# DrSleep/nas-segm-pytorch

Hardware: AMD Instinct MI355X
Metric: images/sec (fwd+bwd+optimizer step) WACV arch0 2048x1024 bs=4/GPU (higher is better)
Workload: dtype f32

## Files before the change

### include/nasseg.h

```cpp
#ifndef NASSEG_H
#define NASSEG_H

#include <stdint.h>

#ifdef __cplusplus
extern "C" {
#endif

const char* nasseg_last_error(void);
int nasseg_abi_version(void);
int nasseg_device_count(void);

int nasseg_dw_pack_weight(const float* w, float* wt, int C, int K, int flip, void* stream);
int nasseg_dwconv(const float* x, const float* wt, float* y, const float* in_scale,
                  const float* in_shift, int in_act, const float* scale, const float* shift, int act,
                  int B, int H, int W, int C, int Ho, int Wo, int K, int stride, int pad, int dil,
                  int transposed, float* stats, void* stream);
int nasseg_dwconv_strip_ok(int K, int stride, int dil);
int64_t nasseg_dwconv_stats_blocks(int B, int C, int Ho, int Wo, int K, int stride, int dil);
int nasseg_dwconv_bwd_data_bn(const float* dy, const float* wt, float* g, const float* z,
                              const float* scale, const float* shift, const float* mean,
                              const float* invstd, int act, int B, int H, int W, int C, int Ho,
                              int Wo, int K, int stride, int pad, int dil, int transposed,
                              float* stats, void* stream);
// ... 7 lines not shown
                         int B, int H, int W, int C, int Ho, int Wo, int K, int stride, int pad, int dil, float* stats,
                         void* stream);
int64_t nasseg_dwconv_wgrad_workspace(int B, int C, int Ho, int Wo, int K);
int nasseg_dwconv_wgrad(const float* x, const float* dy, float* dw, float* ws,
                        const float* in_scale, const float* in_shift, int in_act, int B, int H, int W,
                        int C, int Ho, int Wo, int K, int stride, int pad, int dil, void* stream);

int nasseg_dw_wgrad_lds(int v);

int64_t nasseg_sepconv_blocks(int B, int C, int Ho, int Wo, int N, int K, int stride, int dil);
int nasseg_sepconv_fwd(const float* x, const float* wdw, const float* wpw, float* zdw, float* y,
                       const float* in_scale, const float* in_shift, int in_act,
                       const float* out_scale, const float* out_shift, int out_act, int B, int H,
                       int W, int C, int Ho, int Wo, int N, int K, int stride, int pad, int dil,
                       float* stats, void* stream);

int64_t nasseg_irdw_rows(int B, int H, int W, int K, int C, int stride, int backward);
int64_t nasseg_irdw_config(int B, int H, int W, int K, int C, int stride, int backward);
int64_t nasseg_irdw_stats_workspace(int K);
int nasseg_irdw_stats(const float* x, const float* w1, const float* in_scale, const float* in_shift, int in_act, int B,
                      int H, int W, int K, int C, float eps, float momentum, const float* gamma, const float* beta,
                      float* mean, float* invstd, float* scale, float* shift, float* running_mean, float* running_var,
                      int64_t* num_batches_tracked, float* ws, void* stream);
int nasseg_irdw_fwd(const float* x, const float* w1, const float* wdw, float* z2, const float* in_scale,
                    const float* in_shift, int in_act, const float* bn1_scale, const float* bn1_shift, int act1,
                    int B, int H, int W, int K, int C, int Ho, int Wo, int stride, float* stats, void* stream);
int nasseg_irdw_bwd(const float* x, const float* w1, const float* g, const float* z2, const float* wdw,
                    int wdw_flipped, float* ge, float* dw, float* ws, const float* in_scale, const float* in_shift,
                    int in_act, const float* bn1_scale, const float* bn1_shift, const float* bn1_mean,
                    const float* bn1_invstd, int act1, const float* bn2_scale, const float* bn2_shift,
                    const float* bn2_mean, const float* bn2_invstd, const float* bn2_sums, int bn2_train, int bn2_act,
                    int B, int H, int W, int K, int C, int Ho, int Wo, int stride, float* stats, void* stream);

int nasseg_conv_pack_weight(const float* w, float* wp, int N, int K, int kh, int kw, int mode,
                            void* stream);
int nasseg_pack_weights(int count, const float* const* w, float* const* wp, const int* dims,
                        void* stream);
int nasseg_conv_fwd_pack_mode(int K, int kh, int kw);
int nasseg_conv_fwd(const float* x, int ldx, const float* wp, float* y, int ldy,
                    const float* in_scale, const float* in_shift, int in_act,
                    const float* out_scale, const float* out_shift, int out_act, const float* res,
                    int ldres, int B, int Hs, int Ws, int K, int Ho, int Wo, int N, int kh, int kw,
                    int stride, int pad, int dil, int transposed, float* stats, void* stream);
int64_t nasseg_conv_fwd_stats_blocks(int B, int Ho, int Wo, int N, int K, int pointwise);
int64_t nasseg_conv_fwd_stats_rows(int B, int Ho, int Wo, int N, int K, int kh, int kw, int stride, int pad, int dil);
int64_t nasseg_conv_pw_min_pixels(int64_t v);
int nasseg_conv_pwn_mode(int v);
int nasseg_conv_deep_k(int v);
int nasseg_pool_strip(int v);
int64_t nasseg_conv_pointwise_kernel(int B, int Ho, int Wo, int N, int K, int pointwise);
int64_t nasseg_conv_fwd_lds3x3(int B, int Ho, int Wo, int N, int K, int kh, int kw, int stride, int pad, int dil,
                               int with_stats);
int nasseg_conv_bwd_data_bn(const float* dy, int lddy, const float* wp, float* g, int ldg,
                            const float* z, int ldz, const float* scale, const float* shift,
                            const float* mean, const float* invstd, int act, int B, int Hs, int Ws,
                            int K, int Ho, int Wo, int N, int kh, int kw, int stride, int pad,
                            int dil, float* stats, void* stream);
int nasseg_conv_wgrad_lds3x3(int B, int Hs, int Ws, int K, int Ho, int Wo, int N, int kh, int kw, int stride,
                             int pad, int dil);
int64_t nasseg_conv_wgrad_workspace(int B, int Ho, int Wo, int N, int K, int kh, int kw);
int nasseg_wgrad_finalize_many(int count, const float* const* partial, float* const* dw,
                               const int* dims, void* stream);
int nasseg_conv_wgrad_many(int count, const int64_t* desc, void* stream);
int nasseg_dwconv_wgrad_many(int count, const int64_t* desc, void* stream);

int nasseg_conv_wgrad_bn(const float* x, int ldx, const float* g, int ldg, const float* z, int ldz, float* dz,
                         int lddz, float* dw, float* ws, const float* in_scale, const float* in_shift, int in_act,
                         const float* bn_scale, const float* bn_shift, const float* bn_mean, const float* bn_invstd,
                         const float* bn_sums, int bn_train, int bn_act, int B, int H, int W, int K, int N, void* stream);
int nasseg_conv_wgrad_bn_flat(const float* x, int ldx, const float* g, int ldg, const float* z, int ldz, float* dw,
                              float* ws, const float* bn_scale, const float* bn_shift, const float* bn_mean,
                              const float* bn_invstd, const float* bn_sums, int bn_train, int bn_act, int B, int Hs,
                              int Ws, int K, int Ho, int Wo, int N, int kh, int kw, int stride, int pad, int dil,
                              void* stream);
int nasseg_dwconv_wgrad_bn(const float* x, const float* g, const float* z, float* dz, float* dw, float* ws,
                           const float* in_scale, const float* in_shift, int in_act, const float* bn_scale, const float* bn_shift,
                           const float* bn_mean, const float* bn_invstd, const float* bn_sums, int bn_train, int bn_act,
                           int B, int H, int W, int C, int Ho, int Wo, int K, int stride, int pad, int dil,
                           void* stream);
int64_t nasseg_conv_pw_bwd_slabs(int B, int H, int W, int K, int N);
int64_t nasseg_conv_pw_bwd_reads_z(int B, int H, int W, int K, int N);
int64_t nasseg_conv_pw_bwd_kernel_id(int B, int H, int W, int K, int N, int z_null);
int64_t nasseg_conv_pw_bwd_rz_min_pixels(int64_t v);
int nasseg_conv_pw_bwd_bn(const float* x, const float* g, const float* z, const float* wb, float* dx, float* dw,
                          float* ws, const float* in_scale, const float* in_shift, int in_act, int dx_act,
                          const float* bn_scale, const float* bn_shift, const float* bn_mean, const float* bn_invstd,
                          const float* bn_sums, int bn_train, int bn_act, int B, int H, int W, int K, int N,
                          const float* in_mean, const float* in_invstd, float* dx_stats, const float* dx_res,
                          void* stream);
int nasseg_conv_wgrad(const float* x, int ldx, const float* dy, int lddy, float* dw, float* ws,
                      const float* in_scale, const float* in_shift, int in_act, int B, int Hs,
                      int Ws, int K, int Ho, int Wo, int N, int kh, int kw, int stride, int pad,
                      int dil, void* stream);

int64_t nasseg_colred_workspace(int S, int64_t R, int C);
int nasseg_colred(int mode, const float* a, int64_t lda, const float* b, int64_t ldb,
                  const float* c, int64_t ldc, float* out, float* ws, int S, int64_t R, int C,
                  float mul, void* stream);
int nasseg_bn_stats(const float* x, int64_t ldx, int64_t M, int C, float eps, float momentum,
                    const float* gamma, const float* beta, float* mean, float* invstd,
                    float* scale, float* shift, float* running_mean, float* running_var,
                    int64_t* num_batches_tracked, float* ws, void* stream);
int nasseg_bn_finalize(float* partial, int nblk, int64_t M, int C, float eps, float momentum,
                       const float* gamma, const float* beta, float* mean, float* invstd,
                       float* scale, float* shift, float* running_mean, float* running_var,
                       int64_t* num_batches_tracked, void* stream);
int nasseg_bn_eval_params(int C, float eps, const float* gamma, const float* beta,
                          const float* running_mean, const float* running_var, float* mean,
                          float* invstd, float* scale, float* shift, void* stream);
int nasseg_bn_bwd_reduce(const float* dy, int64_t lddy, const float* x, int64_t ldx, int64_t M,
                         int C, const float* scale, const float* shift, const float* mean,
                         const float* invstd, int act, float* sums, float* ws, void* stream);
int nasseg_rows_sum(float* partial, int nblk, int cols, float* out, void* stream);
int nasseg_bn_bwd_apply(const float* dy, const float* x, const float* scale, const float* shift,
                        const float* mean, const float* invstd, const float* sums, int64_t M,
                        int C, int train, int act, float* dx, void* stream);
int64_t nasseg_colred_rows(int S, int64_t R, int C);
int64_t nasseg_bn_bwd_apply_rows_max_bytes(void);
int nasseg_bn_bwd_reduce_rows(const float* dy, int64_t lddy, const float* x, int64_t ldx, int64_t M, int C,
                              const float* scale, const float* shift, const float* mean, const float* invstd, int act,
                              float* rows, void* stream);
int nasseg_bn_bwd_apply_rows(const float* dy, const float* x, const float* scale, const float* shift, const float* mean,
                             const float* invstd, const float* rows, int nrows, float* sums_out, int64_t M, int C,
                             int train, int act, float* dx, void* stream);

int nasseg_affine_act(const float* x, const float* scale, const float* shift, const float* res,
                      float* y, int64_t n, int C, int act, void* stream);
int nasseg_axpby(const float* a, const float* b, const float* alpha, const float* beta, float* y,
                 int64_t n, int C, int act, void* stream);
int nasseg_add_act2(const float* xa, const float* sa, const float* ha, int act_a, const float* ca, const float* xb,
                    const float* sb, const float* hb, int act_b, const float* cb, float* y, int64_t n, int C,
                    void* stream);
int nasseg_act_bwd(const float* dy, const float* ref, float* dx, int64_t n, int act, void* stream);
int nasseg_fill(float* y, int64_t n, float v, void* stream);
int nasseg_chan_copy(const float* x, int64_t ldx, int xoff, float* y, int64_t ldy, int yoff,
                     const float* mref, int64_t ldm, int moff, int64_t P, int C, int act, int mact,
                     void* stream);
int nasseg_chan_fold(const float* dy, float* dx, int64_t P, int C, int rep, void* stream);
int nasseg_gather_rows(const void* src, const int64_t* idx, void* dst, int n, int64_t row_bytes,
                       int64_t n_src, void* stream);

int nasseg_pool_fwd(int mode, const float* x, float* y, uint8_t* idx, int B, int H, int W, int C,
                    int Ho, int Wo, int K, int stride, int pad, void* stream);
int nasseg_pool_bwd(int mode, const float* dy, const uint8_t* idx, float* dx, int B, int H, int W,
                    int C, int Ho, int Wo, int K, int stride, int pad, void* stream);
int64_t nasseg_maxpool_bn_bwd_blocks(int B, int H, int W, int C, int K, int stride, int pad);
int nasseg_maxpool_bn_fwd(const float* z, const float* scale, const float* shift, float* y, uint8_t* idx,
                          int B, int H, int W, int C, int Ho, int Wo, int stride, int pad, void* stream);
int nasseg_maxpool_bn_bwd(const float* dy, const uint8_t* idx, const float* z, const float* mean,
                          const float* invstd, float* g, float* stats, int B, int H, int W, int C, int Ho,
                          int Wo, int stride, int pad, void* stream);

int64_t nasseg_cat_src_blocks(int B, int Ho, int Wo, int C);
int nasseg_psum_bwd(const float* dy, const float* za, const float* tsa, int act_a, const float* ca, float* ga,
                    float* part_a, const float* zb, const float* tsb, int act_b, const float* cb, float* gb,
                    float* part_b, float* cpart, int B, int H, int W, int C, void* stream);
int nasseg_grad_junction(const float* g0, const float* g1, const float* g2, const float* g3, const float* g4,
                         const float* g5, const float* g6, const float* g7, int n, const float* z, const float* tstats,
                         int act, float* out, float* part, int B, int H, int W, int C, void* stream);
int nasseg_cat_src_fwd(const float* x, const float* scale, const float* shift, int act, float* y, int64_t ldy,
                       int yoff, float* stats, int B, int Hi, int Wi, int C, int Ho, int Wo, void* stream);
int nasseg_cat_src_bwd(const float* du, const float* slab, int64_t ld, int off, const float* sscale,
                       const float* smean, const float* sinvstd, const float* sums, int train, const float* z,
                       const float* tstats, int act, float* g, float* part, int B, int Ho, int Wo, int C, int Hi,
                       int Wi, void* stream);
int nasseg_bilinear_bwd_act(const float* dy, int64_t lddy, int dyoff, const float* z, const float* scale,
// ... 302 lines not shown
```

### nas-segm-pytorch_amd/csrc/conv_pwbwd.hip

```cpp
#include <atomic>
#include <cstdlib>
#include <type_traits>

#include "conv_common.h"

#if NASSEG_FP32_ONLY
std::atomic<int64_t> g_pw_rz_min_pixels{1 << 18};
#else
extern std::atomic<int64_t> g_pw_rz_min_pixels;
#endif

namespace {

#ifndef NASSEG_PW_CHUNK
#define NASSEG_PW_CHUNK 3
#endif
#ifndef NASSEG_PW_RECOMPUTE_Z
#define NASSEG_PW_RECOMPUTE_Z 1
#endif
constexpr int kPwTile = 64;
constexpr int kPwMaxTiles = 24;

struct PwArgs {
  const act_t* x;
  const act_t* g;
  const act_t* z;
  act_t* dx;
  float* partial;
  const float* wb;
  const float* in_scale;
  const float* in_shift;
  int in_act;
  const float* bn_scale;
  const float* bn_shift;
  const float* bn_mean;
  const float* bn_invstd;
  const float* bn_sums;
  int bn_train, bn_act;
  float invM;
  int dx_act;
  const float* in_mean;
  const float* in_invstd;
  float* dx_stats;
  const act_t* dx_res;
  int K, N, KP, NP;
  int M, pix_per_slab;
};

__device__ __forceinline__ float4 act_mask_of(float4 v, int act) {
  const float hi = act == NASSEG_ACT_RELU6 ? 6.f : __builtin_inff();
  return make_float4((v.x > 0.f && v.x < hi) ? 1.f : 0.f, (v.y > 0.f && v.y < hi) ? 1.f : 0.f,
                     (v.z > 0.f && v.z < hi) ? 1.f : 0.f, (v.w > 0.f && v.w < hi) ? 1.f : 0.f);
}

__host__ __device__ constexpr int pw_lsn(int NT) { return NT * 16 + 4; }
__host__ __device__ constexpr int pw_lsk(int KT) { return KT * 16 + 4; }
__host__ __device__ constexpr int pw_lds_floats(int NT, int KT, bool WL) {
  return kPwTile * (pw_lsn(NT) + pw_lsk(KT)) + 4 * NT * 16 + 2 * KT * 16 + (WL ? KT * 16 * pw_lsn(NT) : 0);
}
__host__ __device__ constexpr bool pw_weight_in_lds(int NT, int KT) {
  return pw_lds_floats(NT, KT, true) * 4 <= (72 << 10);
}
__host__ __device__ constexpr bool pw_prefetch(int NT, int KT) { return NT * KT <= 18; }

template <int NT, int KT, bool PRO, bool DXS = false, bool RZ_ = false>
__global__ __launch_bounds__(256) void conv_pw_bwd_kernel(PwArgs a) {
  extern __shared__ float smem[];
  constexpr int LSN = pw_lsn(NT), LSK = pw_lsk(KT), NPc = NT * 16, KPc = KT * 16;
  constexpr bool WL = pw_weight_in_lds(NT, KT), PF = pw_prefetch(NT, KT);
  constexpr bool RZ = WL && RZ_;
  float* dzt = smem;
  float* xt = dzt + kPwTile * LSN;
  float* ca = xt + kPwTile * LSK;
  float* cb = ca + NPc;
  float* cd = cb + NPc;
  float* cs = cd + NPc;
  float* psc = cs + NPc;
  float* psh = psc + KPc;
  float* wl = psh + KPc;
  float* xraw = wl + (WL ? KPc * LSN : 0);
  const int tid = threadIdx.x;
  const int lane = tid & 63, wave = tid >> 6;
  const int j = lane & 15, kg = lane >> 4;
  const int N = a.N, K = a.K;

  for (int n = tid; n < NPc; n += 256) {
    float va = 0.f, vb = 0.f, vd = 0.f, vs = 0.f;
    if (n < N) {
      const float sc = a.bn_scale[n];
      va = sc;
      vs = a.bn_act ? a.bn_shift[n] : 0.f;
      if (a.bn_train) {
        const float is = a.bn_invstd[n], mu = a.bn_mean[n];
        const float s0 = a.bn_sums[n] * a.invM, s1 = a.bn_sums[N + n] * a.invM;
        vb = -sc * is * s1;
        vd = sc * (mu * is * s1 - s0);
      }
    }
    ca[n] = va; cb[n] = vb; cd[n] = vd; cs[n] = vs;
  }
  for (int k = tid; k < KPc; k += 256) {
    psc[k] = (PRO && a.in_scale && k < K) ? a.in_scale[k] : 1.f;
    psh[k] = (PRO && a.in_shift && k < K) ? a.in_shift[k] : 0.f;
  }
  if (WL) {
    for (int it = tid; it < KPc * (NPc / 4); it += 256) {
      const int k = it / (NPc / 4), n = (it - k * (NPc / 4)) * 4;
      const float4 v = keep_if(ld4(a.wb + (int64_t)(k < K ? k : 0) * N + (n < N ? n : 0)), k < K && n < N);
      *reinterpret_cast<float4*>(&wl[k * LSN + n]) = v;
    }
  }
  const ActSel pact = act_sel(a.in_act);

  f32x4 acc2[NT][KT];
#pragma unroll
  for (int nt = 0; nt < NT; ++nt)
#pragma unroll
    for (int kt = 0; kt < KT; ++kt) acc2[nt][kt] = (f32x4){0.f, 0.f, 0.f, 0.f};

  const int p_begin = blockIdx.x * a.pix_per_slab;
  int p_end = p_begin + a.pix_per_slab;
  if (p_end > a.M) p_end = a.M;

  float4 gv[PF ? NT : 1], zv[(PF && !RZ) ? NT : 1], xv[KT];
  auto issue_nz = [&](int t0, int u_lo, int u_hi, float4* G, float4* Z) {
#pragma unroll
    for (int u = 0; u < NT; ++u) {
      if (u < u_lo || u >= u_hi) continue;
      const int it = tid + 256 * u;
      const int px = it / (NPc / 4), n = (it - px * (NPc / 4)) * 4;
      const int p = t0 + px;
      const int64_t off = (int64_t)(p < p_end ? p : p_end - 1) * N + (n < N ? n : 0);
      G[u - u_lo] = lda4(a.g + off);
      if constexpr (!RZ) Z[u - u_lo] = lda4(a.z + off);
    }
  };
  auto issue_x = [&](int t0) {
#pragma unroll
    for (int u = 0; u < KT; ++u) {
      const int it = tid + 256 * u;
      const int px = it / (KPc / 4), k = (it - px * (KPc / 4)) * 4;
      const int p = t0 + px;
      xv[u] = lda4(a.x + (int64_t)(p < p_end ? p : p_end - 1) * K + (k < K ? k : 0));
    }
  };
  auto issue = [&](int t0) {
    issue_nz(t0, 0, NT, gv, zv);
    issue_x(t0);
  };
  auto place_nz = [&](int t0, int u_lo, int u_hi, const float4* G, const float4* Z) {
#pragma unroll
    for (int u = 0; u < NT; ++u) {
      if (u < u_lo || u >= u_hi) continue;
      const int it = tid + 256 * u;
      const int px = it / (NPc / 4), n = (it - px * (NPc / 4)) * 4;
      const bool ok = t0 + px < p_end && n < N;
      if constexpr (RZ) {
        *reinterpret_cast<float4*>(&dzt[px * LSN + n]) = keep_if(G[u - u_lo], ok);
      } else {
        const float4 va = ld4(ca + n), vb = ld4(cb + n), vd = ld4(cd + n);
        float4 g2 = G[u - u_lo];
        const float4 z2 = Z[u - u_lo];
        if (a.bn_act) {
          const float4 y = fma4(z2, va, ld4(cs + n));
          g2 = make_float4(g2.x * act_mask(y.x, a.bn_act), g2.y * act_mask(y.y, a.bn_act),
                           g2.z * act_mask(y.z, a.bn_act), g2.w * act_mask(y.w, a.bn_act));
        }
        float4 dz = fma4(g2, va, fma4(z2, vb, vd));
#ifdef NASSEG_BF16
        dz = make_float4(bf16_to_f32(f32_to_bf16(dz.x)), bf16_to_f32(f32_to_bf16(dz.y)),
                         bf16_to_f32(f32_to_bf16(dz.z)), bf16_to_f32(f32_to_bf16(dz.w)));
#endif
        *reinterpret_cast<float4*>(&dzt[px * LSN + n]) = keep_if(dz, ok);
      }
    }
  };
  float4 sx[DXS ? KT : 1], sq[DXS ? KT : 1], smu[DXS ? KT : 1], sis[DXS ? KT : 1];
#pragma unroll
  for (int kt = 0; kt < (DXS ? KT : 0); ++kt) {
    const int k = kt * 16 + kg * 4;
    sx[kt] = sq[kt] = smu[kt] = sis[kt] = f4zero();
    if (k < K) {
      smu[kt] = lda4(a.in_mean + k);
      sis[kt] = lda4(a.in_invstd + k);
    }
  }
  if (PF && p_begin < p_end) issue(p_begin);
  for (int t0 = p_begin; t0 < p_end; t0 += kPwTile) {
    __syncthreads();
    if (PF) {
      place_nz(t0, 0, NT, gv, zv);
    } else {
      issue_x(t0);
#pragma unroll
      for (int u0 = 0; u0 < NT; u0 += NASSEG_PW_CHUNK) {
        float4 g4[NASSEG_PW_CHUNK], z4[NASSEG_PW_CHUNK];
        issue_nz(t0, u0, u0 + NASSEG_PW_CHUNK, g4, z4);
        place_nz(t0, u0, u0 + NASSEG_PW_CHUNK, g4, z4);
        __builtin_amdgcn_sched_barrier(0);
      }
    }
#pragma unroll
    for (int u = 0; u < KT; ++u) {
      const int it = tid + 256 * u;
      const int px = it / (KPc / 4), k = (it - px * (KPc / 4)) * 4;
      const bool ok = t0 + px < p_end && k < K;
      float4 v = xv[u];
      if (DXS) *reinterpret_cast<float4*>(&xraw[px * LSK + k]) = v;
      if (PRO) v = act_apply4(fma4(v, ld4(psc + k), ld4(psh + k)), pact);
      *reinterpret_cast<float4*>(&xt[px * LSK + k]) = keep_if(v, ok);
    }
    __syncthreads();
    if (PF && t0 + kPwTile < p_end) issue(t0 + kPwTile);
    if constexpr (RZ) {
      constexpr int ZG = NT % 3 == 0 ? 3 : 2;
      const bool pok = t0 + wave * 16 + j < p_end;
      float4 bx[KT];
#pragma unroll
      for (int kb = 0; kb < KT; ++kb)
        bx[kb] = *reinterpret_cast<const float4*>(&xt[(wave * 16 + j) * LSK + kb * 16 + kg * 4]);
#pragma unroll
      for (int n0 = 0; n0 < NT; n0 += ZG) {
        f32x4 zc[ZG];
#pragma unroll
        for (int q = 0; q < ZG; ++q) zc[q] = (f32x4){0.f, 0.f, 0.f, 0.f};
#pragma unroll
        for (int kb = 0; kb < KT; ++kb) {
          const float* wk = wl + (kb * 16 + kg * 4) * LSN + (n0 * 16 + j);
#pragma unroll
          for (int q = 0; q < ZG; ++q) {
            if (n0 + q < NT) {
              zc[q] = mfma16(wk[q * 16], bx[kb].x, zc[q]);
              zc[q] = mfma16(wk[LSN + q * 16], bx[kb].y, zc[q]);
              zc[q] = mfma16(wk[2 * LSN + q * 16], bx[kb].z, zc[q]);
              zc[q] = mfma16(wk[3 * LSN + q * 16], bx[kb].w, zc[q]);
            }
          }
        }
#pragma unroll
        for (int q = 0; q < ZG; ++q) {
          if (n0 + q >= NT) continue;
          const int n = (n0 + q) * 16 + kg * 4;
          float* slot = &dzt[(wave * 16 + j) * LSN + n];
          float4 g2 = *reinterpret_cast<const float4*>(slot);
          float4 z2 = make_float4(zc[q][0], zc[q][1], zc[q][2], zc[q][3]);
#ifdef NASSEG_BF16
          z2 = make_float4(bf16_to_f32(f32_to_bf16(z2.x)), bf16_to_f32(f32_to_bf16(z2.y)), bf16_to_f32(f32_to_bf16(z2.z)),
                           bf16_to_f32(f32_to_bf16(z2.w)));
#endif
          const float4 va = ld4(ca + n), vb = ld4(cb + n), vd = ld4(cd + n);
          if (a.bn_act) {
            const float4 y = fma4(z2, va, ld4(cs + n));
            g2 = make_float4(g2.x * act_mask(y.x, a.bn_act), g2.y * act_mask(y.y, a.bn_act),
                             g2.z * act_mask(y.z, a.bn_act), g2.w * act_mask(y.w, a.bn_act));
          }
          float4 dz = fma4(g2, va, fma4(z2, vb, vd));
#ifdef NASSEG_BF16
          dz = make_float4(bf16_to_f32(f32_to_bf16(dz.x)), bf16_to_f32(f32_to_bf16(dz.y)),
                           bf16_to_f32(f32_to_bf16(dz.z)), bf16_to_f32(f32_to_bf16(dz.w)));
#endif
          *reinterpret_cast<float4*>(slot) = keep_if(dz, pok && n < N);
        }
        __builtin_amdgcn_sched_barrier(0);
      }
    }
    {
      f32x4 acc1[KT];
#pragma unroll
      for (int kt = 0; kt < KT; ++kt) acc1[kt] = (f32x4){0.f, 0.f, 0.f, 0.f};
      float4 rres[KT];
      if (a.dx_res) {
        const int pr = t0 + wave * 16 + j;
#pragma unroll
        for (int kt = 0; kt < KT; ++kt) {
          const int k = kt * 16 + kg * 4;
          rres[kt] = lda4(a.dx_res + ((pr < p_end && k < K) ? (int64_t)pr * K + k : 0));
        }
      }
      const float* brow = dzt + (wave * 16 + j) * LSN;
      for (int ns = 0; ns < (a.NP >> 4); ++ns) {
        const int n = ns * 16 + kg * 4;
        const float4 bv = *reinterpret_cast<const float4*>(brow + n);
        float4 av[KT];
#pragma unroll
        for (int kt = 0; kt < KT; ++kt) {
          const int k = kt * 16 + j;
          if (WL) av[kt] = *reinterpret_cast<const float4*>(&wl[k * LSN + n]);
          else av[kt] = keep_if(ld4(a.wb + (int64_t)(k < K ? k : 0) * N + (n < N ? n : 0)), k < K && n < N);
        }
#pragma unroll
        for (int kt = 0; kt < KT; ++kt) {
          acc1[kt] = mfma16(av[kt].x, bv.x, acc1[kt]);
          acc1[kt] = mfma16(av[kt].y, bv.y, acc1[kt]);
          acc1[kt] = mfma16(av[kt].z, bv.z, acc1[kt]);
          acc1[kt] = mfma16(av[kt].w, bv.w, acc1[kt]);
        }
      }
      const int p = t0 + wave * 16 + j;
#pragma unroll
      for (int kt = 0; kt < KT; ++kt) {
        const int k = kt * 16 + kg * 4;
        float4 o = make_float4(acc1[kt][0], acc1[kt][1], acc1[kt][2], acc1[kt][3]);
        if (a.dx_act)
          o = mul4(o, act_mask_of(*reinterpret_cast<const float4*>(&xt[(wave * 16 + j) * LSK + k]), a.dx_act));
        const bool ok = p < p_end && k < K;
        if (ok) sta4(a.dx + (int64_t)p * K + k, a.dx_res ? add4(o, rres[kt]) : o);
        if (DXS) {
          const float4 zr = *reinterpret_cast<const float4*>(&xraw[(wave * 16 + j) * LSK + k]);
#ifdef NASSEG_BF16
          o = make_float4(bf16_to_f32(f32_to_bf16(o.x)), bf16_to_f32(f32_to_bf16(o.y)), bf16_to_f32(f32_to_bf16(o.z)),
                          bf16_to_f32(f32_to_bf16(o.w)));
#endif
          const float4 gm = keep_if(o, ok);
          const float4 xh = make_float4((zr.x - smu[kt].x) * sis[kt].x, (zr.y - smu[kt].y) * sis[kt].y,
                                        (zr.z - smu[kt].z) * sis[kt].z, (zr.w - smu[kt].w) * sis[kt].w);
          sx[kt] = add4(sx[kt], gm);
          sq[kt] = fma4(gm, xh, sq[kt]);
        }
      }
    }
#pragma unroll
    for (int u = 0; u < 4; ++u) {
      const int pl = wave * 16 + u * 4 + kg;
      float av[NT], bv[KT];
#pragma unroll
      for (int nt = 0; nt < NT; ++nt) av[nt] = dzt[pl * LSN + nt * 16 + j];
#pragma unroll
      for (int kt = 0; kt < KT; ++kt) bv[kt] = xt[pl * LSK + kt * 16 + j];
#pragma unroll
      for (int nt = 0; nt < NT; ++nt)
#pragma unroll
        for (int kt = 0; kt < KT; ++kt) acc2[nt][kt] = mfma16(av[nt], bv[kt], acc2[nt][kt]);
    }
  }

  if (DXS) {
    __syncthreads();
    float* sred = smem;
#pragma unroll
    for (int kt = 0; kt < KT; ++kt) {
      const float vs[4] = {row16_allsum(sx[kt].x), row16_allsum(sx[kt].y), row16_allsum(sx[kt].z), row16_allsum(sx[kt].w)};
      const float vq[4] = {row16_allsum(sq[kt].x), row16_allsum(sq[kt].y), row16_allsum(sq[kt].z), row16_allsum(sq[kt].w)};
      if (j == 0) {
#pragma unroll
        for (int c = 0; c < 4; ++c) {
          sred[(wave * 2 + 0) * KPc + kt * 16 + kg * 4 + c] = vs[c];
          sred[(wave * 2 + 1) * KPc + kt * 16 + kg * 4 + c] = vq[c];
        }
      }
    }
    __syncthreads();
    for (int t = tid; t < KPc; t += 256) {
      if (t < K) {
        float* po = a.dx_stats + (int64_t)blockIdx.x * 2 * K + t;
        po[0] = (sred[0 * KPc + t] + sred[2 * KPc + t]) + (sred[4 * KPc + t] + sred[6 * KPc + t]);
        po[K] = (sred[1 * KPc + t] + sred[3 * KPc + t]) + (sred[5 * KPc + t] + sred[7 * KPc + t]);
      }
    }
  }
  float* red = smem;
  float* pout = a.partial + (int64_t)blockIdx.x * N * K;
#pragma unroll
  for (int nt = 0; nt < NT; ++nt)
#pragma unroll
    for (int kt = 0; kt < KT; ++kt) {
      __syncthreads();
      if (wave > 0) *reinterpret_cast<f32x4*>(&red[((wave - 1) * 64 + lane) * 4]) = acc2[nt][kt];
      __syncthreads();
      if (wave == 0) {
#pragma unroll
        for (int r = 0; r < 4; ++r) {
          const float v = acc2[nt][kt][r] + red[(0 * 64 + lane) * 4 + r] + red[(1 * 64 + lane) * 4 + r] +
                          red[(2 * 64 + lane) * 4 + r];
          const int n = nt * 16 + 4 * kg + r, k = kt * 16 + j;
          if (n < N && k < K) pout[(int64_t)n * K + k] = v;
        }
      }
    }
}

constexpr int kPwChunk = 64;
constexpr int kW2LS = kPwChunk + 4;
template <int KC, bool PRO>
__global__ __launch_bounds__(256, 2) void conv_pw_bwd_wide_kernel(PwArgs a) {
  extern __shared__ float smem[];
  constexpr int LS = kW2LS;
  float* dzt = smem;
  float* xt = dzt + kPwTile * LS;
  float* wt = xt + kPwTile * LS;
  float* wt0 = wt + kPwChunk * LS;
  float* ca = wt0 + kPwChunk * LS;
  float* cb = ca + 64;
  float* cd = cb + 64;
  float* cs = cd + 64;
  float* psc = cs + 64;
  float* psh = psc + KC * kPwChunk;
  const int tid = threadIdx.x;
  const int lane = tid & 63, wave = tid >> 6;
  const int j = lane & 15, kg = lane >> 4;
  const int N = a.N, K = a.K;
  for (int n = tid; n < 64; n += 256) {
    float va = 0.f, vb = 0.f, vd = 0.f, vs = 0.f;
    if (n < N) {
      const float sc = a.bn_scale[n];
      va = sc;
      vs = a.bn_act ? a.bn_shift[n] : 0.f;
      if (a.bn_train) {
        const float is = a.bn_invstd[n], mu = a.bn_mean[n];
        const float s0 = a.bn_sums[n] * a.invM, s1 = a.bn_sums[N + n] * a.invM;
        vb = -sc * is * s1;
        vd = sc * (mu * is * s1 - s0);
      }
    }
    ca[n] = va; cb[n] = vb; cd[n] = vd; cs[n] = vs;
  }
  for (int k = tid; k < KC * kPwChunk; k += 256) {
    psc[k] = (PRO && a.in_scale && k < K) ? a.in_scale[k] : 1.f;
    psh[k] = (PRO && a.in_shift && k < K) ? a.in_shift[k] : 0.f;
  }
  const ActSel pact = act_sel(a.in_act);
  f32x4 acc2[KC][4];
#pragma unroll
  for (int c = 0; c < KC; ++c)
#pragma unroll
    for (int q = 0; q < 4; ++q) acc2[c][q] = (f32x4){0.f, 0.f, 0.f, 0.f};
  const int p_begin = blockIdx.x * a.pix_per_slab;
  int p_end = p_begin + a.pix_per_slab;
  if (p_end > a.M) p_end = a.M;
  const bool own = wave * 16 < a.NP;
  const int NS = a.NP >> 4;
  const float m_lo = a.bn_act ? 0.f : -__builtin_inff();
  const float m_hi = a.bn_act == NASSEG_ACT_RELU6 ? 6.f : __builtin_inff();
  const int irow = tid >> 4, icol = (tid & 15) * 4;
  float4 XN[4], WN[4], GN[4], ZN[4];
  auto issue_gz = [&](int t0) {
#pragma unroll
    for (int u = 0; u < 4; ++u) {
      const int p = t0 + irow + 16 * u;
      const int64_t off = (int64_t)(p < p_end ? p : p_end - 1) * N + (icol < N ? icol : 0);
      GN[u] = lda4(a.g + off);
      ZN[u] = lda4(a.z + off);
    }
  };
  auto issue_xw = [&](int t0, int kc) {
    const int k = kc + icol;
#pragma unroll
    for (int u = 0; u < 4; ++u) {
      const int p = t0 + irow + 16 * u;
      XN[u] = lda4(a.x + (int64_t)(p < p_end ? p : p_end - 1) * K + (k < K ? k : 0));
      if (kc) {
        const int kw = kc + irow + 16 * u;
        WN[u] = ld4(a.wb + (int64_t)(kw < K ? kw : 0) * N + (icol < N ? icol : 0));
      }
    }
  };
  auto place_gz = [&](int t0) {
    const float4 va = ld4(ca + icol), vb = ld4(cb + icol), vd = ld4(cd + icol), vs = ld4(cs + icol);
#pragma unroll
    for (int u = 0; u < 4; ++u) {
      const int px = irow + 16 * u;
      const bool ok = t0 + px < p_end && icol < N;
// ... 127 lines not shown
  }
  if (own) {
    float* pout = a.partial + (int64_t)blockIdx.x * N * K;
#pragma unroll
    for (int c = 0; c < KC; ++c)
#pragma unroll
      for (int q = 0; q < 4; ++q)
#pragma unroll
        for (int r = 0; r < 4; ++r) {
          const int n = wave * 16 + 4 * kg + r, k = c * kPwChunk + q * 16 + j;
          if (n < N && k < K) pout[(int64_t)n * K + k] = acc2[c][q][r];
        }
  }
}

struct PwPlan {
  int ok, nt, kt, nslab, pix_per_slab, wide, rz;
};
inline int pw_round_nt(int nt) {
  const int allowed[] = {2, 3, 4, 6, 9, 12};
  for (int v : allowed)
    if (nt <= v) return v;
  return 0;
}
inline PwPlan pw_plan(int64_t M, int N, int K) {
  PwPlan p = {};
  if (N % 4 || K % 4 || N <= 0 || K <= 0 || M <= 0 || M >= 2147483647LL) return p;
  const int kt0 = cdiv(K, 16);
  p.kt = kt0 <= 1 ? 1 : (kt0 <= 2 ? 2 : (kt0 <= 4 ? 4 : 0));
  p.nt = pw_round_nt(cdiv(N, 16));
  if (!p.kt || !p.nt || p.nt * p.kt > kPwMaxTiles) {
    if (N > 64 || K > 384) return p;
    p.wide = 1;
    p.nt = cdiv(N, 16);
    p.kt = cdiv(K, kPwChunk);
  }
  const int64_t lds = p.wide ? (int64_t)(32 << 10)
                             : (int64_t)pw_lds_floats(p.nt, p.kt, pw_weight_in_lds(p.nt, p.kt)) * 4;
  int64_t s = lds > (40 << 10) ? 512 : 1024;
  const int64_t cap = (int64_t)((p.wide ? 64 : 16) << 20) / ((int64_t)N * K * 4);
  while (s > 1 && (s > cap || s > M / (4 * kPwTile))) s >>= 1;
  if (!p.wide && s < 256 && M / kPwTile > s) {
    s = M / kPwTile < 256 ? M / kPwTile : 256;
    if (s > cap) s = cap;
    if (s < 1) s = 1;
  }
#ifdef NASSEG_TUNE
  if (const char* e = getenv("NASSEG_PW_SLABS")) {
    const int64_t v = atoll(e);
    if (v > 0 && v <= cap) s = v;
  }
#endif
  int64_t ppb = cdiv64(M, s);
  ppb = (ppb + kPwTile - 1) / kPwTile * kPwTile;
  p.pix_per_slab = (int)ppb;
  p.nslab = (int)cdiv64(M, ppb);
  p.rz = NASSEG_PW_RECOMPUTE_Z != 0 && !p.wide && p.kt <= 2 && p.nt <= 6 && pw_weight_in_lds(p.nt, p.kt) &&
         M >= g_pw_rz_min_pixels.load();
  p.ok = 1;
  return p;
}

#define PW_NARROW(X) \
  X(2, 1) X(3, 1) X(4, 1) X(6, 1) X(9, 1) X(12, 1) X(2, 2) X(3, 2) X(4, 2) X(6, 2) X(9, 2) X(12, 2) X(2, 4) X(3, 4) X(4, 4) X(6, 4)
#define PW_REBUILD(X) X(2, 1) X(3, 1) X(4, 1) X(6, 1) X(2, 2) X(3, 2) X(4, 2) X(6, 2) X(9, 2)
constexpr int kPwIdWide = 10000;
constexpr int pw_id(int nt, int kt, int rz) { return nt * 100 + kt * 10 + rz; }
inline int pw_kernel_id(const PwPlan& p, bool z_null) {
  if (!p.ok) return -1;
  if (p.wide) return (z_null || p.kt > 6) ? -1 : kPwIdWide + (p.kt <= 2 ? 2 : p.kt);
  const int id = pw_id(p.nt, p.kt, (p.rz || z_null) ? 1 : 0);
  switch (id) {
#define X(NT_, KT_) case pw_id(NT_, KT_, 1):
    PW_REBUILD(X)
#undef X
#define X(NT_, KT_) case pw_id(NT_, KT_, 0):
    PW_NARROW(X)
#undef X
      return id;
    default: return -1;
  }
}

template <int NT, int KT, bool RZ = false>
void pw_launch(const PwArgs& a, int nslab, bool pro, hipStream_t s) {
  static_assert(!RZ || pw_weight_in_lds(NT, KT), "the kernel rebuilds z only with its weight in LDS: it would read a.z");
  constexpr size_t lds = (size_t)pw_lds_floats(NT, KT, pw_weight_in_lds(NT, KT)) * sizeof(float);
  constexpr size_t lds_dxs = lds + (size_t)kPwTile * pw_lsk(KT) * sizeof(float);
  if (lds_dxs > (64 << 10)) {
    (void)hipFuncSetAttribute((const void*)conv_pw_bwd_kernel<NT, KT, true, true, RZ>,
                              hipFuncAttributeMaxDynamicSharedMemorySize, (int)lds_dxs);
    if (pro) (void)hipFuncSetAttribute((const void*)conv_pw_bwd_kernel<NT, KT, true, false, RZ>,
                                       hipFuncAttributeMaxDynamicSharedMemorySize, (int)lds);
    else (void)hipFuncSetAttribute((const void*)conv_pw_bwd_kernel<NT, KT, false, false, RZ>,
                                   hipFuncAttributeMaxDynamicSharedMemorySize, (int)lds);
  }
  if (a.dx_stats) hipLaunchKernelGGL((conv_pw_bwd_kernel<NT, KT, true, true, RZ>), dim3(nslab), dim3(256), lds_dxs, s, a);
  else if (pro) hipLaunchKernelGGL((conv_pw_bwd_kernel<NT, KT, true, false, RZ>), dim3(nslab), dim3(256), lds, s, a);
  else hipLaunchKernelGGL((conv_pw_bwd_kernel<NT, KT, false, false, RZ>), dim3(nslab), dim3(256), lds, s, a);
}

}

extern "C" {

#if NASSEG_FP32_ONLY
int64_t nasseg_conv_pw_bwd_slabs(int B, int H, int W, int K, int N) {
  const PwPlan p = pw_plan((int64_t)B * H * W, N, K);
  return p.ok ? p.nslab : 0;
}
#endif

#if NASSEG_FP32_ONLY
int64_t nasseg_conv_pw_bwd_reads_z(int B, int H, int W, int K, int N) {
  const PwPlan p = pw_plan((int64_t)B * H * W, N, K);
  return (p.ok && p.rz) ? 0 : 1;
}
int64_t nasseg_conv_pw_bwd_kernel_id(int B, int H, int W, int K, int N, int z_null) {
  if (B <= 0 || H <= 0 || W <= 0) return -1;
  return pw_kernel_id(pw_plan((int64_t)B * H * W, N, K), z_null != 0);
}
int64_t nasseg_conv_pw_bwd_rz_min_pixels(int64_t v) {
  if (v < 0) return g_pw_rz_min_pixels.load();
  return g_pw_rz_min_pixels.exchange(v);
}
#endif

int NASSEG_FN(conv_pw_bwd_bn)(const act_t* x, const act_t* g, const act_t* z, const float* wb, act_t* dx,
                              float* dw, float* ws, const float* in_scale, const float* in_shift,
                              int in_act, int dx_act, const float* bn_scale, const float* bn_shift,
                              const float* bn_mean, const float* bn_invstd, const float* bn_sums,
                              int bn_train, int bn_act, int B, int H, int W, int K, int N, const float* in_mean,
                              const float* in_invstd, float* dx_stats, const act_t* dx_res, void* stream) {
  NASSEG_REQUIRE(x && g && wb && dx && ws && bn_scale, "conv_pw_bwd_bn: null tensor");
  NASSEG_REQUIRE(!dx_stats || (in_mean && in_invstd), "conv_pw_bwd_bn: dx_stats needs in_mean / in_invstd");
  NASSEG_REQUIRE(!dx_res || (!dx_stats && K % 4 == 0), "conv_pw_bwd_bn: dx_res needs K %% 4 == 0 and no dx_stats");
  NASSEG_REQUIRE((!bn_train || (bn_mean && bn_invstd && bn_sums)) && (!bn_act || bn_shift),
                 "conv_pw_bwd_bn: missing BatchNorm tensors");
  NASSEG_REQUIRE(B > 0 && H > 0 && W > 0, "conv_pw_bwd_bn: bad geometry");
  const int64_t M = (int64_t)B * H * W;
  const PwPlan p = pw_plan(M, N, K);
  NASSEG_REQUIRE(p.ok, "conv_pw_bwd_bn: no fused kernel for K=%d N=%d", K, N);
  const int id = pw_kernel_id(p, !z);
  NASSEG_REQUIRE(z || id >= 0, "conv_pw_bwd_bn: z == NULL, but K=%d N=%d has no kernel that rebuilds z", K, N);
  if (id < 0)
    return nasseg_fail(NASSEG_ERR_UNSUPPORTED, "conv_pw_bwd_bn: no kernel for nt=%d kt=%d rz=%d", p.nt, p.kt, p.rz);
  PwArgs a = {};
  a.x = x; a.g = g; a.z = z; a.dx = dx; a.partial = ws; a.wb = wb;
  a.in_scale = in_scale; a.in_shift = in_shift; a.in_act = in_act;
  a.bn_scale = bn_scale; a.bn_shift = bn_shift; a.bn_mean = bn_mean; a.bn_invstd = bn_invstd;
  a.bn_sums = bn_sums; a.bn_train = bn_train; a.bn_act = bn_act;
  a.invM = (float)(1.0 / (double)M);
  NASSEG_REQUIRE(!dx_act || dx_act == in_act,
                 "conv_pw_bwd_bn: dx can only be masked with the derivative of the input activation");
  a.dx_act = dx_act;
  a.in_mean = in_mean; a.in_invstd = in_invstd; a.dx_stats = dx_stats; a.dx_res = dx_res;
  a.K = K; a.N = N; a.KP = (K + 15) & ~15; a.NP = (N + 15) & ~15;
  a.M = (int)M; a.pix_per_slab = p.pix_per_slab;
  const bool pro = in_scale || in_shift || in_act;
  hipStream_t s = (hipStream_t)stream;
  if (p.wide) {
    NASSEG_REQUIRE(!dx_stats, "conv_pw_bwd_bn: dx_stats is not available for K > 64");
    const size_t ldsw2 = ((size_t)4 * kPwTile * kW2LS + 4 * 64 + 2 * p.kt * kPwChunk) * sizeof(float);
#define PW_WIDE(KC_)                                                                                         \
  do {                                                                                                       \
    if (ldsw2 > (64 << 10)) {  \
      (void)hipFuncSetAttribute((const void*)conv_pw_bwd_wide_kernel<KC_, true>,                            \
                                hipFuncAttributeMaxDynamicSharedMemorySize, (int)ldsw2);                     \
      (void)hipFuncSetAttribute((const void*)conv_pw_bwd_wide_kernel<KC_, false>,                           \
                                hipFuncAttributeMaxDynamicSharedMemorySize, (int)ldsw2);                     \
    }                                                                                                        \
    if (pro) hipLaunchKernelGGL((conv_pw_bwd_wide_kernel<KC_, true>), dim3(p.nslab), dim3(256), ldsw2, s, a); \
    else hipLaunchKernelGGL((conv_pw_bwd_wide_kernel<KC_, false>), dim3(p.nslab), dim3(256), ldsw2, s, a);    \
  } while (0)
    switch (id - kPwIdWide) {
      case 2: PW_WIDE(2); break;
      case 3: PW_WIDE(3); break;
      case 4: PW_WIDE(4); break;
      case 5: PW_WIDE(5); break;
      case 6: PW_WIDE(6); break;
      default: return nasseg_fail(NASSEG_ERR_UNSUPPORTED, "conv_pw_bwd_bn: no kernel with id %d", id);
    }
#undef PW_WIDE
    NASSEG_LAUNCH_CHECK("conv_pw_bwd_wide_kernel");
    if (!dw) return NASSEG_OK;
    const float* parts_w[1] = {ws};
    float* outs_w[1] = {dw};
    const int dims_w[5] = {p.nslab, 1, N, K, 0};
    return nasseg_wgrad_finalize_many(1, parts_w, outs_w, dims_w, stream);
  }
  switch (id) {
#define X(NT_, KT_) case pw_id(NT_, KT_, 1): pw_launch<NT_, KT_, true>(a, p.nslab, pro, s); break;
    PW_REBUILD(X)
#undef X
#define X(NT_, KT_) case pw_id(NT_, KT_, 0): pw_launch<NT_, KT_>(a, p.nslab, pro, s); break;
    PW_NARROW(X)
#undef X
    default: return nasseg_fail(NASSEG_ERR_UNSUPPORTED, "conv_pw_bwd_bn: no kernel with id %d", id);
  }
  NASSEG_LAUNCH_CHECK("conv_pw_bwd_kernel");
  if (!dw) return NASSEG_OK;
  const float* parts[1] = {ws};
  float* outs[1] = {dw};
  const int dims[5] = {p.nslab, 1, N, K, 0};
  return nasseg_wgrad_finalize_many(1, parts, outs, dims, stream);
}

}
```

### nas-segm-pytorch_amd/functional.py

```python
import collections
import ctypes
import os
import weakref

import numpy as np
import torch

from ._lib import LaunchProfiler, NassegError, current_stream, lib, ptr, require_device

ACT_NONE, ACT_RELU, ACT_RELU6 = 0, 1, 2
RED_SUM, RED_SUMSQ, RED_DOT2, RED_DOT1 = 0, 1, 3, 4


_BF16_PREFIX = "nasseg_bf16_"


def _k(name, t):
    if t.dtype == torch.float32:
        return name
    return _BF16_PREFIX + name[7:]


def _to_dtype(t, dtype):
    if t.dtype == dtype:
# ... 2615 lines not shown
                name, (n_classes, n_classes)))
    else:
        cm = None
    dev = first.device
    labels = torch.empty((B, H, W), device=dev, dtype=torch.uint8) if want_labels else None
    probs = (torch.empty((B, C, H, W), device=dev, dtype=torch.float32, memory_format=torch.channels_last)
             if want_probs else None)
    mean = (torch.empty((B, C, H, W), device=dev, dtype=torch.float32, memory_format=torch.channels_last)
            if want_mean else None)
    table = (ctypes.c_void_p * len(views))(*[ptr(v) for v in views])
    hdims = (ctypes.c_int * (3 * len(views)))(*[int(d) for d in dims.ravel()])
    if lib.recorder is not None:
        lib.recorder.annotate(reads=views + [taps, coef, gt], writes=[labels, probs, cm, mean])
    lib.call(_k("nasseg_fuse_views", first), len(views), table, hdims, ptr(taps), ptr(coef), T, B, C, H, W, ptr(gt),
             n_classes if cm is not None else 0, ptr(labels), ptr(probs), ptr(cm), ptr(mean), current_stream())
    return labels, probs, cm, mean


def fuse_views(views, size, mirrored, mode="cubic", gt=None, n_classes=None, cm=None, return_probs=False,
               tables=None, return_mean=False):
    labels, probs, cm, mean = _fuse("fuse_views", views, size, mirrored, mode, tables, gt, n_classes, cm, True,
                                    return_probs, return_mean)
    out = ([cm] if gt is not None else []) + [labels] + ([probs] if return_probs else []) + (
        [mean] if return_mean else [])
    return out[0] if len(out) == 1 else tuple(out)


def fuse_views_mean(views, size, mirrored, mode="cubic", tables=None):
    return _fuse("fuse_views_mean", views, size, mirrored, mode, tables, None, None, None, False, False, True)[3]


def prepare_plan(device, B, H, W, dtype=torch.float32):
    import numpy as np

    from .data import device as ddev

    if dtype not in (torch.float32, torch.bfloat16):
        raise NassegError("prepare_image: images are float32 or bfloat16 (got {})".format(dtype))

    def make():
        axes = []
        for n in (H, W):
            c = np.arange(n, dtype=np.int64)
            axes.append((np.concatenate([np.repeat(c[:, None], 4, axis=1),
                                         np.broadcast_to(ddev._IDENTITY_COEF, (n, 4))], 1), c))
        (ty, my), (tx, mx) = axes
        taps = np.concatenate([ty.ravel(), tx.ravel(), my, mx]).astype(np.int32)
        desc = np.zeros((B, ddev.DESC_FIELDS), np.int64)
        desc[:, 0] = np.arange(B, dtype=np.int64) * (H * W * 3)
        desc[:, 2:6] = (H, W, 3 * W, W)
        lut = torch.from_numpy(ddev.prepare_img_table()).float().to(dtype)
        return (torch.from_numpy(desc).to(device), torch.from_numpy(np.tile(taps, (B, 1))).to(device),
                lut.to(device))

    return _lru(_PREPARE_PLANS, (torch.device(device), int(B), int(H), int(W), dtype), make)


def prepare_image(img, dtype=torch.float32, plan=None):
    require_device(img)
    if img.dtype != torch.uint8 or img.dim() != 4 or img.shape[3] != 3 or img.numel() == 0:
        raise NassegError("prepare_image: expected a uint8 B x H x W x 3 image (got {} {})".format(
            img.dtype, tuple(img.shape)))
    B, H, W, _ = img.shape
    img = img.contiguous()
    desc, taps, lut = plan if plan is not None else prepare_plan(img.device, B, H, W, dtype)
    if (lut.dtype != dtype or tuple(desc.shape) != (B, 8) or tuple(taps.shape) != (B, 9 * (H + W))
            or desc.device != img.device):
        raise NassegError("prepare_image: the plan does not match a {} batch of {}x{}".format(B, H, W))
    image = torch.empty((B, 3, H, W), device=img.device, dtype=dtype, memory_format=torch.channels_last)
    lib.call(_k("nasseg_augment", image), ptr(img), img.numel(), ptr(desc), ptr(taps), ptr(lut), ptr(image), None,
             B, H, W, current_stream())
    return image


def _apply_library_knobs():
    if _PW_MIN_PIXELS is not None:
        lib.query("nasseg_conv_pw_min_pixels", int(_PW_MIN_PIXELS))
        lib._memo.clear()
    if _PWN_MODE is not None:
        lib.query("nasseg_conv_pwn_mode", int(_PWN_MODE))
        lib._memo.clear()
    for env, fn in (("NASSEG_DW_WGRAD_LDS", "nasseg_dw_wgrad_lds"), ("NASSEG_CONV_DEEP_K", "nasseg_conv_deep_k"),
                    ("NASSEG_POOL_STRIP", "nasseg_pool_strip"),
                    ("NASSEG_PW_RZ_MIN_PIXELS", "nasseg_conv_pw_bwd_rz_min_pixels")):
        if os.environ.get(env) is not None:
            lib.query(fn, int(os.environ[env]))
            lib._memo.clear()


try:
    _apply_library_knobs()
except (OSError, NassegError):
    pass
```

Baseline: 308.3.

## Split pointwise-conv backward weight-grad accumulation across waves by output channel

```diff
diff --git a/include/nasseg.h b/include/nasseg.h
--- a/include/nasseg.h
+++ b/include/nasseg.h
@@ -113,6 +113,7 @@
 int64_t nasseg_conv_pw_bwd_reads_z(int B, int H, int W, int K, int N);
 int64_t nasseg_conv_pw_bwd_kernel_id(int B, int H, int W, int K, int N, int z_null);
 int64_t nasseg_conv_pw_bwd_rz_min_pixels(int64_t v);
+int nasseg_conv_pw_bwd_nsplit(int v);
 int nasseg_conv_pw_bwd_bn(const float* x, const float* g, const float* z, const float* wb, float* dx, float* dw,
                           float* ws, const float* in_scale, const float* in_shift, int in_act, int dx_act,
                           const float* bn_scale, const float* bn_shift, const float* bn_mean, const float* bn_invstd,
diff --git a/nas-segm-pytorch_amd/csrc/conv_pwbwd.hip b/nas-segm-pytorch_amd/csrc/conv_pwbwd.hip
--- a/nas-segm-pytorch_amd/csrc/conv_pwbwd.hip
+++ b/nas-segm-pytorch_amd/csrc/conv_pwbwd.hip
@@ -9,6 +9,11 @@
 #else
 extern std::atomic<int64_t> g_pw_rz_min_pixels;
 #endif
+#if NASSEG_FP32_ONLY
+std::atomic<int> g_pw_nsplit{1};
+#else
+extern std::atomic<int> g_pw_nsplit;
+#endif
 
 namespace {
 
@@ -17,6 +22,9 @@
 #endif
 #ifndef NASSEG_PW_RECOMPUTE_Z
 #define NASSEG_PW_RECOMPUTE_Z 1
+#endif
+#ifndef NASSEG_PW_NSPLIT
+#define NASSEG_PW_NSPLIT 1
 #endif
 constexpr int kPwTile = 64;
 constexpr int kPwMaxTiles = 24;
@@ -61,13 +69,20 @@
 __host__ __device__ constexpr bool pw_weight_in_lds(int NT, int KT) {
   return pw_lds_floats(NT, KT, true) * 4 <= (72 << 10);
 }
-__host__ __device__ constexpr bool pw_prefetch(int NT, int KT) { return NT * KT <= 18; }
-
-template <int NT, int KT, bool PRO, bool DXS = false, bool RZ_ = false>
-__global__ __launch_bounds__(256) void conv_pw_bwd_kernel(PwArgs a) {
+__host__ __device__ constexpr bool pw_prefetch(int NT, int KT, bool NS = false) { return NS || NT * KT <= 18; }
+
+__host__ __device__ constexpr bool pw_two_waves(int NT, int KT, bool DXS, bool NS) {
+  return NS && NT >= 9 && !(NT * KT >= 24 && DXS);
+}
+
+template <int NT, int KT, bool PRO, bool DXS = false, bool RZ_ = false, bool NS_ = false>
+__global__ __launch_bounds__(256, pw_two_waves(NT, KT, DXS, NS_) ? 2 : 1) void conv_pw_bwd_kernel(PwArgs a) {
   extern __shared__ float smem[];
   constexpr int LSN = pw_lsn(NT), LSK = pw_lsk(KT), NPc = NT * 16, KPc = KT * 16;
-  constexpr bool WL = pw_weight_in_lds(NT, KT), PF = pw_prefetch(NT, KT);
+  constexpr bool NS = NS_ && NT >= 9;
+  constexpr int NTW = NS ? (NT + 3) / 4 : NT;
+  constexpr bool WL = pw_weight_in_lds(NT, KT), PF = pw_prefetch(NT, KT, NS);
+  constexpr bool PF_LATE = PF && !WL;
   constexpr bool RZ = WL && RZ_;
   float* dzt = smem;
   float* xt = dzt + kPwTile * LSN;
@@ -112,9 +127,9 @@
   }
   const ActSel pact = act_sel(a.in_act);
 
-  f32x4 acc2[NT][KT];
-#pragma unroll
-  for (int nt = 0; nt < NT; ++nt)
+  f32x4 acc2[NTW][KT];
+#pragma unroll
+  for (int nt = 0; nt < NTW; ++nt)
 #pragma unroll
     for (int kt = 0; kt < KT; ++kt) acc2[nt][kt] = (f32x4){0.f, 0.f, 0.f, 0.f};
 
@@ -211,7 +226,7 @@
       *reinterpret_cast<float4*>(&xt[px * LSK + k]) = keep_if(v, ok);
     }
     __syncthreads();
-    if (PF && t0 + kPwTile < p_end) issue(t0 + kPwTile);
+    if (PF && !PF_LATE && t0 + kPwTile < p_end) issue(t0 + kPwTile);
     if constexpr (RZ) {
       constexpr int ZG = NT % 3 == 0 ? 3 : 2;
       const bool pok = t0 + wave * 16 + j < p_end;
@@ -319,18 +334,40 @@
         }
       }
     }
-#pragma unroll
-    for (int u = 0; u < 4; ++u) {
-      const int pl = wave * 16 + u * 4 + kg;
-      float av[NT], bv[KT];
-#pragma unroll
-      for (int nt = 0; nt < NT; ++nt) av[nt] = dzt[pl * LSN + nt * 16 + j];
-#pragma unroll
-      for (int kt = 0; kt < KT; ++kt) bv[kt] = xt[pl * LSK + kt * 16 + j];
-#pragma unroll
-      for (int nt = 0; nt < NT; ++nt)
-#pragma unroll
-        for (int kt = 0; kt < KT; ++kt) acc2[nt][kt] = mfma16(av[nt], bv[kt], acc2[nt][kt]);
+    if (PF_LATE && t0 + kPwTile < p_end) issue(t0 + kPwTile);
+    if constexpr (NS) {
+      if constexpr (RZ) __syncthreads();
+      const int w0 = __builtin_amdgcn_readfirstlane(wave);
+#pragma unroll 4
+      for (int u = 0; u < kPwTile / 4; ++u) {
+        const int pl = u * 4 + kg;
+        float av[NTW], bv[KT];
+#pragma unroll
+        for (int i = 0; i < NTW; ++i)
+          if (NT % 4 == 0 || w0 + 4 * i < NT) av[i] = dzt[pl * LSN + (w0 + 4 * i) * 16 + j];
+#pragma unroll
+        for (int kt = 0; kt < KT; ++kt) bv[kt] = xt[pl * LSK + kt * 16 + j];
+#pragma unroll
+        for (int i = 0; i < NTW; ++i)
+          if (NT % 4 == 0 || w0 + 4 * i < NT) {
+#pragma unroll
+            for (int kt = 0; kt < KT; ++kt) acc2[i][kt] = mfma16(av[i], bv[kt], acc2[i][kt]);
+          }
+      }
+    } else {
+#pragma unroll
+      for (int u = 0; u < 4; ++u) {
+        const int pl = wave * 16 + u * 4 + kg;
+        float av[NT], bv[KT];
+#pragma unroll
+        for (int nt = 0; nt < NT; ++nt) av[nt] = dzt[pl * LSN + nt * 16 + j];
+#pragma unroll
+        for (int kt = 0; kt < KT; ++kt) bv[kt] = xt[pl * LSK + kt * 16 + j];
+#pragma unroll
+        for (int nt = 0; nt < NT; ++nt)
+#pragma unroll
+          for (int kt = 0; kt < KT; ++kt) acc2[nt][kt] = mfma16(av[nt], bv[kt], acc2[nt][kt]);
+      }
     }
   }
 
@@ -358,25 +395,38 @@
       }
     }
   }
-  float* red = smem;
   float* pout = a.partial + (int64_t)blockIdx.x * N * K;
-#pragma unroll
-  for (int nt = 0; nt < NT; ++nt)
-#pragma unroll
-    for (int kt = 0; kt < KT; ++kt) {
-      __syncthreads();
-      if (wave > 0) *reinterpret_cast<f32x4*>(&red[((wave - 1) * 64 + lane) * 4]) = acc2[nt][kt];
-      __syncthreads();
-      if (wave == 0) {
+  if constexpr (NS) {
+    const int w0 = __builtin_amdgcn_readfirstlane(wave);
+#pragma unroll
+    for (int i = 0; i < NTW; ++i)
+#pragma unroll
+      for (int kt = 0; kt < KT; ++kt)
 #pragma unroll
         for (int r = 0; r < 4; ++r) {
-          const float v = acc2[nt][kt][r] + red[(0 * 64 + lane) * 4 + r] + red[(1 * 64 + lane) * 4 + r] +
-                          red[(2 * 64 + lane) * 4 + r];
-          const int n = nt * 16 + 4 * kg + r, k = kt * 16 + j;
-          if (n < N && k < K) pout[(int64_t)n * K + k] = v;
-        }
-      }
-    }
+          const int n = (w0 + 4 * i) * 16 + 4 * kg + r, k = kt * 16 + j;
+          if (n < N && k < K) pout[(int64_t)n * K + k] = acc2[i][kt][r];
+        }
+  } else {
+    float* red = smem;
+#pragma unroll
+    for (int nt = 0; nt < NT; ++nt)
+#pragma unroll
+      for (int kt = 0; kt < KT; ++kt) {
+        __syncthreads();
+        if (wave > 0) *reinterpret_cast<f32x4*>(&red[((wave - 1) * 64 + lane) * 4]) = acc2[nt][kt];
+        __syncthreads();
+        if (wave == 0) {
+#pragma unroll
+          for (int r = 0; r < 4; ++r) {
+            const float v = acc2[nt][kt][r] + red[(0 * 64 + lane) * 4 + r] + red[(1 * 64 + lane) * 4 + r] +
+                            red[(2 * 64 + lane) * 4 + r];
+            const int n = nt * 16 + 4 * kg + r, k = kt * 16 + j;
+            if (n < N && k < K) pout[(int64_t)n * K + k] = v;
+          }
+        }
+      }
+  }
 }
 
 constexpr int kPwChunk = 64;
@@ -670,22 +720,39 @@
   }
 }
 
-template <int NT, int KT, bool RZ = false>
+inline bool pw_nsplit(int id) {
+  const int mode = NASSEG_PW_NSPLIT ? g_pw_nsplit.load() : 0;
+  if (id < 0 || id >= kPwIdWide || id / 100 < 9 || mode <= 0) return false;
+  if (mode >= 2) return true;
+  switch (id) {
+    case pw_id(9, 2, 0): case pw_id(9, 2, 1): case pw_id(12, 1, 0): case pw_id(12, 2, 0): return true;
+    default: return false;
+  }
+}
+
+template <int NT, int KT, bool RZ = false, bool NS = false>
 void pw_launch(const PwArgs& a, int nslab, bool pro, hipStream_t s) {
   static_assert(!RZ || pw_weight_in_lds(NT, KT), "the kernel rebuilds z only with its weight in LDS: it would read a.z");
   constexpr size_t lds = (size_t)pw_lds_floats(NT, KT, pw_weight_in_lds(NT, KT)) * sizeof(float);
   constexpr size_t lds_dxs = lds + (size_t)kPwTile * pw_lsk(KT) * sizeof(float);
   if (lds_dxs > (64 << 10)) {
-    (void)hipFuncSetAttribute((const void*)conv_pw_bwd_kernel<NT, KT, true, true, RZ>,
+    (void)hipFuncSetAttribute((const void*)conv_pw_bwd_kernel<NT, KT, true, true, RZ, NS>,
                               hipFuncAttributeMaxDynamicSharedMemorySize, (int)lds_dxs);
-    if (pro) (void)hipFuncSetAttribute((const void*)conv_pw_bwd_kernel<NT, KT, true, false, RZ>,
+    if (pro) (void)hipFuncSetAttribute((const void*)conv_pw_bwd_kernel<NT, KT, true, false, RZ, NS>,
                                        hipFuncAttributeMaxDynamicSharedMemorySize, (int)lds);
-    else (void)hipFuncSetAttribute((const void*)conv_pw_bwd_kernel<NT, KT, false, false, RZ>,
+    else (void)hipFuncSetAttribute((const void*)conv_pw_bwd_kernel<NT, KT, false, false, RZ, NS>,
                                    hipFuncAttributeMaxDynamicSharedMemorySize, (int)lds);
   }
-  if (a.dx_stats) hipLaunchKernelGGL((conv_pw_bwd_kernel<NT, KT, true, true, RZ>), dim3(nslab), dim3(256), lds_dxs, s, a);
-  else if (pro) hipLaunchKernelGGL((conv_pw_bwd_kernel<NT, KT, true, false, RZ>), dim3(nslab), dim3(256), lds, s, a);
-  else hipLaunchKernelGGL((conv_pw_bwd_kernel<NT, KT, false, false, RZ>), dim3(nslab), dim3(256), lds, s, a);
+  if (a.dx_stats) hipLaunchKernelGGL((conv_pw_bwd_kernel<NT, KT, true, true, RZ, NS>), dim3(nslab), dim3(256), lds_dxs, s, a);
+  else if (pro) hipLaunchKernelGGL((conv_pw_bwd_kernel<NT, KT, true, false, RZ, NS>), dim3(nslab), dim3(256), lds, s, a);
+  else hipLaunchKernelGGL((conv_pw_bwd_kernel<NT, KT, false, false, RZ, NS>), dim3(nslab), dim3(256), lds, s, a);
+}
+template <int NT, int KT, bool RZ>
+void pw_launch_id(const PwArgs& a, int nslab, bool pro, bool ns, hipStream_t s) {
+  if constexpr (NASSEG_PW_NSPLIT != 0 && NT >= 9) {
+    if (ns) return pw_launch<NT, KT, RZ, true>(a, nslab, pro, s);
+  }
+  pw_launch<NT, KT, RZ>(a, nslab, pro, s);
 }
 
 }
@@ -711,6 +778,10 @@
 int64_t nasseg_conv_pw_bwd_rz_min_pixels(int64_t v) {
   if (v < 0) return g_pw_rz_min_pixels.load();
   return g_pw_rz_min_pixels.exchange(v);
+}
+int nasseg_conv_pw_bwd_nsplit(int v) {
+  if (v < 0) return g_pw_nsplit.load();
+  return g_pw_nsplit.exchange(v > 2 ? 2 : v);
 }
 #endif
 
@@ -778,10 +849,10 @@
     return nasseg_wgrad_finalize_many(1, parts_w, outs_w, dims_w, stream);
   }
   switch (id) {
-#define X(NT_, KT_) case pw_id(NT_, KT_, 1): pw_launch<NT_, KT_, true>(a, p.nslab, pro, s); break;
+#define X(NT_, KT_) case pw_id(NT_, KT_, 1): pw_launch_id<NT_, KT_, true>(a, p.nslab, pro, pw_nsplit(id), s); break;
     PW_REBUILD(X)
 #undef X
-#define X(NT_, KT_) case pw_id(NT_, KT_, 0): pw_launch<NT_, KT_>(a, p.nslab, pro, s); break;
+#define X(NT_, KT_) case pw_id(NT_, KT_, 0): pw_launch_id<NT_, KT_, false>(a, p.nslab, pro, pw_nsplit(id), s); break;
     PW_NARROW(X)
 #undef X
     default: return nasseg_fail(NASSEG_ERR_UNSUPPORTED, "conv_pw_bwd_bn: no kernel with id %d", id);
diff --git a/nas-segm-pytorch_amd/functional.py b/nas-segm-pytorch_amd/functional.py
--- a/nas-segm-pytorch_amd/functional.py
+++ b/nas-segm-pytorch_amd/functional.py
@@ -2721,7 +2721,8 @@
         lib._memo.clear()
     for env, fn in (("NASSEG_DW_WGRAD_LDS", "nasseg_dw_wgrad_lds"), ("NASSEG_CONV_DEEP_K", "nasseg_conv_deep_k"),
                     ("NASSEG_POOL_STRIP", "nasseg_pool_strip"),
-                    ("NASSEG_PW_RZ_MIN_PIXELS", "nasseg_conv_pw_bwd_rz_min_pixels")):
+                    ("NASSEG_PW_RZ_MIN_PIXELS", "nasseg_conv_pw_bwd_rz_min_pixels"),
+                    ("NASSEG_PW_NSPLIT", "nasseg_conv_pw_bwd_nsplit")):
         if os.environ.get(env) is not None:
             lib.query(fn, int(os.environ[env]))
             lib._memo.clear()
```

New measurement: 311.3, median of 6. No clear change (+1.0%).
